# lh3/bwa

Measured on NVIDIA H100. Metric: reads_per_sec, higher is better.
Workload: dtype int32

## Files before the change

### bwa_b200/csrc/cuda/bwag_api.cu

```cuda
#include <stdio.h>
#include <stdlib.h>
#include <string.h>
#include <stdarg.h>
#include <pthread.h>
#include <time.h>
#include <math.h>
#include <sched.h>
#include "bwag_dev.cuh"
#include "bwag_kernels.h"

struct BlobHeader {
	u64 magic, primary, seq_len, bwt_size, n_sa, l_pac;
	u64 L2[5];
	u64 sa_shift;
	u64 off_bwt, off_sa, off_pac, total;
	u64 sb[BWAG_MAX_SB][4];
};
#define BLOB_MAGIC 0x3142574142323030ull
#define ALIGN256(x) (((x) + 255) & ~(size_t)255)

static __thread char g_err[512];
extern "C" const char *bwag_last_error(void) { return g_err[0] ? g_err : "no error"; }
static int set_err(const char *fmt, ...)
{
	va_list ap;
	va_start(ap, fmt);
	vsnprintf(g_err, sizeof(g_err), fmt, ap);
	va_end(ap);
	return 1;
}
int bwag_set_error(const char *msg) { return set_err("%s", msg); }
#define CK(call) do { cudaError_t e_ = (call); if (e_ != cudaSuccess) return set_err("%s failed at %s:%d: %s", #call, __FILE__, __LINE__, cudaGetErrorString(e_)); } while (0)
#define CKP(call) do { cudaError_t e_ = (call); if (e_ != cudaSuccess) { set_err("%s failed at %s:%d: %s", #call, __FILE__, __LINE__, cudaGetErrorString(e_)); return 0; } } while (0)

struct Counters {
	int next_read, next_task, max_rlen, next_read3;
	u64 next_seed;
	u64 n_intv, n_seeds;
	u64 occ_touches, sa_touches, ext_cells, glb_cells;
	u64 n_cig, n_md;
	u32 flags, n_pre;
	u64 t_dregs, t_tasks, t_max_z, t_text, t_complex;
	int t_max_lq, t_max_rl;
	int n_many;
	u32 n_swtasks;
};

struct DevBuf { void *p; size_t cap; };
static int buf_reserve(DevBuf *b, size_t bytes)
{
	if (bytes <= b->cap) return 0;
	if (b->p) cudaFree(b->p);
	b->p = 0; b->cap = 0;
	size_t want = bytes + bytes / 4 + 256;
	CK(cudaMalloc(&b->p, want));
	b->cap = want;
	return 0;
}
struct HostBuf { void *p; size_t cap; };
static int hbuf_reserve(HostBuf *b, size_t bytes)
{
	if (bytes <= b->cap) return 0;
	if (b->p) cudaFreeHost(b->p);
	b->p = 0; b->cap = 0;
	size_t want = bytes + bytes / 4 + 256;
	CK(cudaMallocHost(&b->p, want));
	b->cap = want;
	return 0;
}

struct bwag_ctx {
	int device, own_blob, n_sm;
	int imported;
	size_t map_bytes[3];
	void *blob;
	DevIndex ix;
	u64 *dense_sa;
	ulonglong2 *ktab;
	int baseline;
	cudaStream_t stream;
	cudaEvent_t ev0, ev1, ev_wait;
	Counters *d_cnt, *h_cnt;
	bwag_stats_t st;
	int sa_intv_disk;
	DevBuf s_k1, s_k1f, s_n3, s_eh, s_rseq, s_qseq, s_z, s_wcig, s_wmd, s_pack, s_zl;
	int grid_k1, grid_k1f, grid_k2, grid_k4, grid_k5;
#define N_SPARE 12
	struct bwag_batch *spare[N_SPARE];
	pthread_mutex_t mu;
	struct bwag_ctx *parent;
	void *d_tail; TailCtg tctg; const double *d_logtab; int have_ctg;
};

struct bwag_batch {
	bwag_ctx_t *ctx;
	bwag_ctx_t lc;
	int lc_ready;
	int n;
	i64 total_bases;
	int max_len;
	const i64 *h_off;
	DevBuf d_codes, d_off;
	DevBuf d_intv_beg, d_intv_n, d_intv, d_seed_beg, d_rbeg;
	HostBuf h_intv_beg, h_intv_n, h_intv, h_seed_beg, h_rbeg;
	DevBuf d_chain_off, d_chains, d_seeds, d_regs, d_nregs;
	DevBuf d_chain_beg, d_chain_cnt, d_reg_base, d_chain_rid, d_chain_frac, d_cregs, d_creg_beg, d_ctg;
	DevBuf s_bt, s_sn, s_ch, s_order, s_idx, s_keys;
	HostBuf h_regs, h_nregs, h_cregs, h_creg_beg, h_tmp;
	i64 n_intv, n_seeds;
	int seeded;
	DevBuf d_tasks, d_res, d_cig, d_md;
	HostBuf h_res, h_cig, h_md;
	DevBuf d_dregs, d_dreg_beg, d_dreg_n, d_task_beg, d_cflag, d_pe_is, d_rec, d_text, d_ptab;
	DevBuf d_swtasks, d_swres, d_swpool, d_swscratch; HostBuf h_swres;
	DevBuf d_hsp, d_flt_nchn; HostBuf h_hsp;
	DevBuf d_pre_n, d_pre_score, d_pre_cig;
	DevBuf d_sel;
	HostBuf h_pe_is, h_cflag, h_rec, h_text, h_ptab;
	int tail_ready;
	int regs_on_device;
};

static void batch_free(bwag_batch_t *b);
static void free_dev(DevBuf *b) { if (b->p) cudaFree(b->p); b->p = 0; b->cap = 0; }
static void free_host(HostBuf *b) { if (b->p) cudaFreeHost(b->p); b->p = 0; b->cap = 0; }

#ifndef BWAG_L2_FETCH_DEFAULT
#define BWAG_L2_FETCH_DEFAULT 0
#endif
#define K1_SMEM_MAX (200 * 1024)
#ifndef K1_COMPACT_DEFAULT
#define K1_COMPACT_DEFAULT 1
#endif
#ifdef BWAG_CUSIM
#define BWAG_KTAB_MAX_AUTO 5
#else
#define BWAG_KTAB_MAX_AUTO 14
#endif
#define K4_SMEM_MAX (96 * 1024)
#define K4L_SMEM_MAX (200 * 1024)
#define SEEDSW_MAXLEN 200

#ifdef BWAG_CUSIM
unsigned long long bwag_cusim_sector_loads, bwag_cusim_list_acc[5];
#endif


extern "C" size_t bwag_blob_bytes(const bwt_t *bwt, int64_t l_pac)
{
	return ALIGN256(sizeof(BlobHeader)) + ALIGN256((size_t)bwt->bwt_size * 4 + 64) + ALIGN256((size_t)bwt->n_sa * 8 + 32) + ALIGN256((size_t)l_pac / 4 + 1 + 64);
}

extern "C" int bwag_blob_fill(int device, void *d_blob, const bwt_t *bwt, int64_t l_pac, const uint8_t *pac)
{
	BlobHeader h;
	if (device >= 0) CK(cudaSetDevice(device));
	memset(&h, 0, sizeof(h));
	h.magic = BLOB_MAGIC; h.primary = bwt->primary; h.seq_len = bwt->seq_len; h.bwt_size = bwt->bwt_size; h.n_sa = bwt->n_sa; h.l_pac = (u64)l_pac;
	for (int i = 0; i < 5; ++i) h.L2[i] = bwt->L2[i];
	{
		int s = 0;
		while ((1 << s) < bwt->sa_intv) ++s;
		if ((1 << s) != bwt->sa_intv) return set_err("suffix-array interval %d is not a power of two", bwt->sa_intv);
		h.sa_shift = (u64)s;
	}
	if (bwt->seq_len >= (u64)BWAG_MAX_SB << BWAG_SB_SHIFT) return set_err("index too large: %llu BWT symbols", (unsigned long long)bwt->seq_len);
	for (u64 s = 0; s << BWAG_SB_SHIFT < bwt->seq_len; ++s) {
		const u64 *cnt = (const u64 *)(bwt->bwt + ((s << BWAG_SB_SHIFT) >> 7) * 16);
		for (int k = 0; k < 4; ++k) h.sb[s][k] = cnt[k];
// ... 400 lines not shown
	CKP(cudaMemcpyAsync(b->d_off.p, off, sizeof(i64) * ((size_t)n + 1), cudaMemcpyHostToDevice, c->stream));
	c->st.h2d_bytes += (u64)b->total_bases + sizeof(i64) * ((u64)n + 1);
	CKP(cudaEventRecord(c->ev1, c->stream));
	CKP(cudaStreamSynchronize(c->stream));
	{ float ms = 0; cudaEventElapsedTime(&ms, c->ev0, c->ev1); c->st.ms_h2d += ms; }
	return b;
}

extern "C" void bwag_batch_end(bwag_batch_t *b)
{
	if (!b) return;
	bwag_ctx_t *c = b->ctx;
	cudaSetDevice(c->device);
	cudaStreamSynchronize(b->lc.stream);
	pthread_mutex_lock(&c->mu);
	{
		bwag_stats_t *d = &c->st, *x = &b->lc.st;
		d->occ_touches += x->occ_touches; d->sa_touches += x->sa_touches; d->sa_touches_algo += x->sa_touches_algo;
		d->ext_cells += x->ext_cells; d->glb_cells += x->glb_cells;
		d->ms_smem += x->ms_smem; d->ms_sa += x->ms_sa; d->ms_chain += x->ms_chain; d->ms_extend += x->ms_extend; d->ms_global += x->ms_global;
		d->ms_h2d += x->ms_h2d; d->ms_d2h += x->ms_d2h; d->n_launch += x->n_launch; d->h2d_bytes += x->h2d_bytes; d->d2h_bytes += x->d2h_bytes;
		d->ms_tail += x->ms_tail; d->tail_reads += x->tail_reads; d->tail_complex += x->tail_complex; d->ms_localsw += x->ms_localsw; d->sw_tasks += x->sw_tasks;
	}
#ifdef BWAG_CUSIM
	if (getenv("BWA_B200_PROFILE")) fprintf(stderr, "[prof] emulator: %llu 32-byte block/table loads so far (K1, K1f, K2, table build); K1 candidate-list accesses by entry index 0-3: %llu, 4-7: %llu, 8-11: %llu, 12-15: %llu, 16+: %llu (the first K1_SLOTS of a list live in shared memory)\n", bwag_cusim_sector_loads, bwag_cusim_list_acc[0], bwag_cusim_list_acc[1], bwag_cusim_list_acc[2], bwag_cusim_list_acc[3], bwag_cusim_list_acc[4]);
#endif
	if (getenv("BWA_B200_PROFILE"))
		fprintf(stderr, "[prof] batch counters: %d reads, occ_touches %llu, sa_touches %llu, ext_cells %llu, glb_cells %llu; stage 4: %llu reads, %llu handed back to the host-side post-processing; K6: %llu local alignments\n", b->n,
		        (unsigned long long)b->lc.st.occ_touches, (unsigned long long)b->lc.st.sa_touches, (unsigned long long)b->lc.st.ext_cells, (unsigned long long)b->lc.st.glb_cells,
		        (unsigned long long)b->lc.st.tail_reads, (unsigned long long)b->lc.st.tail_complex, (unsigned long long)b->lc.st.sw_tasks);
	for (int i = 0; i < N_SPARE; ++i) if (!c->spare[i]) { c->spare[i] = b; b = 0; break; }
	pthread_mutex_unlock(&c->mu);
	if (b) batch_free(b);
}

static void batch_free(bwag_batch_t *b)
{
	if (b->lc_ready) {
		free_dev(&b->lc.s_pack); free_dev(&b->lc.s_k1); free_dev(&b->lc.s_k1f); free_dev(&b->lc.s_n3); free_dev(&b->lc.s_eh); free_dev(&b->lc.s_rseq); free_dev(&b->lc.s_qseq); free_dev(&b->lc.s_z); free_dev(&b->lc.s_wcig); free_dev(&b->lc.s_wmd);
		cudaFree(b->lc.d_cnt); cudaFreeHost(b->lc.h_cnt);
		cudaEventDestroy(b->lc.ev0); cudaEventDestroy(b->lc.ev1); cudaEventDestroy(b->lc.ev_wait); cudaStreamDestroy(b->lc.stream);
	}
	free_dev(&b->d_codes); free_dev(&b->d_off);
	free_dev(&b->d_intv_beg); free_dev(&b->d_intv_n); free_dev(&b->d_intv); free_dev(&b->d_seed_beg); free_dev(&b->d_rbeg);
	free_host(&b->h_intv_beg); free_host(&b->h_intv_n); free_host(&b->h_intv); free_host(&b->h_seed_beg); free_host(&b->h_rbeg);
	free_dev(&b->d_chain_off); free_dev(&b->d_chains); free_dev(&b->d_seeds); free_dev(&b->d_regs); free_dev(&b->d_nregs);
	free_dev(&b->d_chain_beg); free_dev(&b->d_chain_cnt); free_dev(&b->d_reg_base); free_dev(&b->d_chain_rid); free_dev(&b->d_chain_frac); free_dev(&b->d_cregs); free_dev(&b->d_creg_beg); free_dev(&b->d_ctg);
	free_dev(&b->s_bt); free_dev(&b->s_sn); free_dev(&b->s_ch); free_dev(&b->s_order); free_dev(&b->s_idx); free_dev(&b->s_keys);
	free_host(&b->h_regs); free_host(&b->h_nregs); free_host(&b->h_cregs); free_host(&b->h_creg_beg); free_host(&b->h_tmp);
	free_dev(&b->d_tasks); free_dev(&b->d_res); free_dev(&b->d_cig); free_dev(&b->d_md);
	free_host(&b->h_res); free_host(&b->h_cig); free_host(&b->h_md);
	free_dev(&b->d_sel); free_dev(&b->d_swtasks); free_dev(&b->d_swres); free_dev(&b->d_swpool); free_dev(&b->d_swscratch); free_host(&b->h_swres);
	free_dev(&b->d_hsp); free_dev(&b->d_flt_nchn); free_host(&b->h_hsp);
	free_dev(&b->d_pre_n); free_dev(&b->d_pre_score); free_dev(&b->d_pre_cig);
	free_dev(&b->d_dregs); free_dev(&b->d_dreg_beg); free_dev(&b->d_dreg_n); free_dev(&b->d_task_beg); free_dev(&b->d_cflag); free_dev(&b->d_pe_is); free_dev(&b->d_rec); free_dev(&b->d_text); free_dev(&b->d_ptab);
	free_host(&b->h_pe_is); free_host(&b->h_cflag); free_host(&b->h_rec); free_host(&b->h_text); free_host(&b->h_ptab);
	free(b);
}

static int reset_counters(bwag_ctx_t *c)
{
	CK(cudaMemsetAsync(c->d_cnt, 0, sizeof(Counters), c->stream));
	return 0;
}
static cudaError_t stream_wait(bwag_ctx_t *c)
{
	static int mode = -1;
	if (mode < 0) { const char *e = getenv("BWA_B200_SYNC"); mode = !e ? 3 : strcmp(e, "spin") == 0 ? 0 : strcmp(e, "block") == 0 ? 1 : strcmp(e, "yield") == 0 ? 2 : 3; }
	if (mode == 0) return cudaStreamSynchronize(c->stream);
	if (mode == 3) {
		long ns = 5000;
		for (;;) {
			cudaError_t q = cudaStreamQuery(c->stream);
			if (q != cudaErrorNotReady) return q;
			struct timespec ts = { 0, ns };
			nanosleep(&ts, 0);
			if (ns < 80000) ns <<= 1;
		}
	}
	if (mode == 2) {
		for (;;) {
			cudaError_t q = cudaStreamQuery(c->stream);
			if (q != cudaErrorNotReady) return q;
			sched_yield();
		}
	}
	cudaError_t e = cudaEventRecord(c->ev_wait, c->stream);
	if (e != cudaSuccess) return e;
	return cudaEventSynchronize(c->ev_wait);
}

static int fetch_counters(bwag_ctx_t *c)
{
	CK(cudaMemcpyAsync(c->h_cnt, c->d_cnt, sizeof(Counters), cudaMemcpyDeviceToHost, c->stream));
	CK(stream_wait(c));
	return 0;
}
#define H2D(c, dst, src, bytes) do { CK(cudaMemcpyAsync((dst), (src), (bytes), cudaMemcpyHostToDevice, (c)->stream)); (c)->st.h2d_bytes += (u64)(bytes); } while (0)
#define D2H(c, dst, src, bytes) do { CK(cudaMemcpyAsync((dst), (src), (bytes), cudaMemcpyDeviceToHost, (c)->stream)); (c)->st.d2h_bytes += (u64)(bytes); } while (0)
static double elapsed_at(bwag_ctx_t *c, const char *stage, int line)
{
	float ms = 0;
	cudaEventElapsedTime(&ms, c->ev0, c->ev1);
	if (g_gputrace > 0) {
		float t0 = 0, t1 = 0;
		cudaEventElapsedTime(&t0, g_trace_ref, c->ev0); cudaEventElapsedTime(&t1, g_trace_ref, c->ev1);
		fprintf(stderr, "[gputrace] %p %s:%d %.3f %.3f\n", (void *)c, stage, line, t0, t1);
// ... 505 lines not shown
	c->st.ms_d2h += elapsed_at(c, "d2h", __LINE__);
	out->n_regs = (const int32_t *)b->h_nregs.p; out->reg_beg = (const int64_t *)b->h_creg_beg.p; out->regs = (const bwag_creg_t *)b->h_cregs.p;
	return 0;
}


static int run_global(bwag_batch_t *b, const bwag_sw_par_t *par, int n_tasks, int cap_q, int cap_r, i64 cap_z, i64 n_aln, i64 *nc_out, i64 *nm_out)
{
	bwag_ctx_t *c = &b->lc;
	cap_q = (cap_q + 3) & ~3; cap_r = (cap_r + 15) & ~15; cap_z = (cap_z + 15) & ~(i64)15;
	if (cap_q < 4) cap_q = 4;
	if (cap_r < 16) cap_r = 16;
	if (cap_z < 64) cap_z = 64;
	const int cap_wcig = cap_q + cap_r + 4, cap_wmd = 3 * cap_r + cap_q + 16;
	int grid = c->grid_k5;
	const int k5_zsm = getenv("BWA_B200_K5_ZSM") ? atoi(getenv("BWA_B200_K5_ZSM")) & ~15 : 6144;
	const int k5_per_warp = ((8 * (cap_q + 2) + cap_r + cap_q + 2 + 15) & ~15) + k5_zsm;
	const size_t k5_smem = (size_t)k5_per_warp * (K5_THREADS / 32);
	int k5_sm = k5_smem <= K4_SMEM_MAX && !(getenv("BWA_B200_K5_SM") && atoi(getenv("BWA_B200_K5_SM")) == 0);
	const int k5_fast = !c->baseline && !(getenv("BWA_B200_K5_FAST") && atoi(getenv("BWA_B200_K5_FAST")) == 0);
#ifndef BWAG_CUSIM
	if (k5_sm) { int nb = 0; CK(cudaOccupancyMaxActiveBlocksPerMultiprocessor(&nb, k5_fast ? k_global_sm_fast : k_global_sm, K5_THREADS, k5_smem)); if (nb < 2) k5_sm = 0; else grid = c->n_sm * nb; }
#endif
	{
		i64 need = ((i64)n_tasks + (K5_THREADS / 32) - 1) / (K5_THREADS / 32);
		if (grid > need) grid = (int)(need > 0 ? need : 1);
		i64 max_warps = ((i64)8 << 30) / cap_z;
		if (max_warps < K5_THREADS / 32) max_warps = K5_THREADS / 32;
		if ((i64)grid * (K5_THREADS / 32) > max_warps) grid = (int)(max_warps / (K5_THREADS / 32));
	}
	const size_t n_warps = (size_t)grid * (K5_THREADS / 32);
	if (buf_reserve(&c->s_eh, n_warps * 2 * (size_t)(cap_q + 2) * 4) || buf_reserve(&c->s_rseq, n_warps * (size_t)cap_r) ||
	    buf_reserve(&c->s_qseq, n_warps * (size_t)(cap_q + 2)) || buf_reserve(&c->s_z, n_warps * (size_t)cap_z) ||
	    buf_reserve(&c->s_wcig, n_warps * (size_t)cap_wcig * 4) || buf_reserve(&c->s_wmd, n_warps * (size_t)cap_wmd)) return 1;
	if (buf_reserve(&b->d_res, sizeof(bwag_gres_t) * (size_t)n_tasks)) return 1;
	int k5_lane = !c->baseline && cap_q <= K5L_QWORDS * 4 && n_tasks >= 64 && getenv("BWA_B200_K5_LANE") && atoi(getenv("BWA_B200_K5_LANE")) != 0;
	const size_t k5l_smem = (size_t)K5L_RING * K5L_THREADS * 8 + (size_t)K5L_QWORDS * K5L_THREADS * 4;
	const i64 k5l_cap_z = (i64)(K5L_RING - 1) * (cap_r < 1024 ? cap_r : 1024);
	int k5l_grid = 0;
	if (k5_lane) {
#ifndef BWAG_CUSIM
		int nb = 0;
		CK(cudaFuncSetAttribute(k_global_lane, cudaFuncAttributeMaxDynamicSharedMemorySize, (int)k5l_smem));
		CK(cudaOccupancyMaxActiveBlocksPerMultiprocessor(&nb, k_global_lane, K5L_THREADS, k5l_smem));
		k5l_grid = c->n_sm * (nb > 0 ? nb : 1);
#else
		k5l_grid = 2;
#endif
		const i64 need = ((i64)n_tasks + K5L_THREADS - 1) / K5L_THREADS;
		if (k5l_grid > need) k5l_grid = (int)need;
		if (buf_reserve(&b->d_pre_n, 4 * (size_t)n_tasks) || buf_reserve(&b->d_pre_score, 4 * (size_t)n_tasks) || buf_reserve(&b->d_pre_cig, 4 * (size_t)K5L_MAXCIG * (size_t)n_tasks) ||
		    buf_reserve(&c->s_zl, (size_t)k5l_cap_z * (size_t)k5l_grid * K5L_THREADS)) return 1;
	}
	i64 cap_cig = n_aln * 6 + 1024, cap_md = n_aln * 24 + 4096;
	for (int attempt = 0;; ++attempt) {
		if (buf_reserve(&b->d_cig, 4 * (size_t)cap_cig) || buf_reserve(&b->d_md, (size_t)cap_md)) return 1;
		GlbArgs a;
		memset(&a, 0, sizeof(a));
		a.codes = (const uint8_t *)b->d_codes.p; a.off = (const i64 *)b->d_off.p; a.par = *par;
		a.tasks = (const bwag_gtask_t *)b->d_tasks.p; a.n_tasks = n_tasks;
		a.res = (bwag_gres_t *)b->d_res.p; a.cigar = (u32 *)b->d_cig.p; a.md = (char *)b->d_md.p;
		a.cap_cig = cap_cig; a.cap_md = cap_md; a.n_cig = &c->d_cnt->n_cig; a.n_md = &c->d_cnt->n_md;
		a.w_cig = (u32 *)c->s_wcig.p; a.w_md = (char *)c->s_wmd.p; a.cap_wcig = cap_wcig; a.cap_wmd = cap_wmd;
		a.eh = (int *)c->s_eh.p; a.rseq = (uint8_t *)c->s_rseq.p; a.qseq = (uint8_t *)c->s_qseq.p; a.z = (uint8_t *)c->s_z.p;
		a.cap_q = cap_q; a.cap_r = cap_r; a.cap_z = cap_z;
		a.next_task = &c->d_cnt->next_task; a.cells = &c->d_cnt->glb_cells; a.flags = &c->d_cnt->flags;
		if (reset_counters(c)) return 1;
		CK(cudaEventRecord(c->ev0, c->stream));
		if (k5_lane) {
			GlbLaneArgs la;
			memset(&la, 0, sizeof(la));
			la.codes = a.codes; la.off = a.off; la.par = *par; la.tasks = a.tasks; la.n_tasks = n_tasks;
			la.pre_n = (int *)b->d_pre_n.p; la.pre_score = (int *)b->d_pre_score.p; la.pre_cig = (u32 *)b->d_pre_cig.p;
			la.z = (uint8_t *)c->s_zl.p; la.cap_z = k5l_cap_z; la.next_task = &c->d_cnt->next_task; la.cells = &c->d_cnt->glb_cells; la.n_pre = &c->d_cnt->n_pre;
			BWAG_LAUNCH(k_global_lane, k5l_grid, K5L_THREADS, k5l_smem, c->stream, c->ix, la);
			CK(cudaGetLastError());
			CK(cudaMemsetAsync(&c->d_cnt->next_task, 0, sizeof(int), c->stream));
			a.pre_n = la.pre_n; a.pre_score = la.pre_score; a.pre_cig = la.pre_cig;
			++c->st.n_launch;
		}
		a.smem_per_warp = k5_sm ? k5_per_warp : 0; a.z_sm_bytes = k5_sm ? k5_zsm : 0;
		if (k5_sm && k5_fast) BWAG_LAUNCH(k_global_sm_fast, grid, K5_THREADS, k5_smem, c->stream, c->ix, a);
		else if (k5_sm) BWAG_LAUNCH(k_global_sm, grid, K5_THREADS, k5_smem, c->stream, c->ix, a);
		else if (k5_fast) BWAG_LAUNCH(k_global_fast, grid, K5_THREADS, 0, c->stream, c->ix, a);
		else BWAG_LAUNCH(k_global, grid, K5_THREADS, 0, c->stream, c->ix, a);
		CK(cudaGetLastError());
		CK(cudaEventRecord(c->ev1, c->stream));
		if (fetch_counters(c)) return 1;
		c->st.ms_global += elapsed_at(c, "global", __LINE__); ++c->st.n_launch;
		if (k5_lane && getenv("BWA_B200_PROFILE")) fprintf(stderr, "[prof] global alignment: lane-per-request kernel made %u of %d CIGARs, grid %d x %d\n", c->h_cnt->n_pre, n_tasks, k5l_grid, K5L_THREADS);
		if (c->h_cnt->flags & 4u) return set_err("global alignment: a task exceeded the scratch capacity");
		if (!(c->h_cnt->flags & 16u)) break;
		if (attempt >= 3) return set_err("global alignment: output pools keep overflowing");
		cap_cig = (i64)c->h_cnt->n_cig + 1024; cap_md = (i64)c->h_cnt->n_md + 4096;
	}
	c->st.glb_cells += c->h_cnt->glb_cells;
	*nc_out = (i64)c->h_cnt->n_cig; *nm_out = (i64)c->h_cnt->n_md;
	return 0;
}

extern "C" int bwag_global(bwag_batch_t *b, const bwag_sw_par_t *par, int n_tasks, const bwag_gtask_t *tasks, bwag_galn_t *out)
{
	bwag_ctx_t *c = &b->lc;
	CK(cudaSetDevice(c->device));
	if (n_tasks <= 0) { out->res = 0; out->cigar = 0; out->md = 0; return 0; }
	i64 cap_z = 64, n_aln = 0, nc = 0, nm = 0;
	int cap_q = 4, cap_r = 16;
	for (int t = 0; t < n_tasks; ++t) {
		i64 lq = tasks[t].qe - tasks[t].qb, rl = tasks[t].re - tasks[t].rb;
		if (lq > cap_q) cap_q = (int)lq;
		if (rl > cap_r) cap_r = (int)rl;
		if (tasks[t].mode == BWAG_G_REG2ALN) {
			i64 d = rl > lq ? rl - lq : lq - rl, wmax = (i64)par->w << 2;
			if (d + 3 > wmax) wmax = d + 3;
			i64 ncol = lq < 2 * wmax + 1 ? lq : 2 * wmax + 1;
			if (ncol * rl > cap_z) cap_z = ncol * rl;
			++n_aln;
		}
	}
	if (buf_reserve(&b->d_tasks, sizeof(bwag_gtask_t) * (size_t)n_tasks)) return 1;
	CK(cudaEventRecord(c->ev0, c->stream));
	H2D(c, b->d_tasks.p, tasks, sizeof(bwag_gtask_t) * (size_t)n_tasks);
	CK(cudaEventRecord(c->ev1, c->stream));
	CK(stream_wait(c));
	c->st.ms_h2d += elapsed_at(c, "h2d", __LINE__);
	b->tail_ready = 0;
	if (run_global(b, par, n_tasks, cap_q, cap_r, cap_z, n_aln, &nc, &nm)) return 1;
	if (hbuf_reserve(&b->h_res, sizeof(bwag_gres_t) * (size_t)n_tasks) || hbuf_reserve(&b->h_cig, 4 * (size_t)(nc + 1)) || hbuf_reserve(&b->h_md, (size_t)nm + 16)) return 1;
	CK(cudaEventRecord(c->ev0, c->stream));
	D2H(c, b->h_res.p, b->d_res.p, sizeof(bwag_gres_t) * (size_t)n_tasks);
	if (nc) D2H(c, b->h_cig.p, b->d_cig.p, 4 * (size_t)nc);
	if (nm) D2H(c, b->h_md.p, b->d_md.p, (size_t)nm);
	CK(cudaEventRecord(c->ev1, c->stream));
	CK(stream_wait(c));
	c->st.ms_d2h += elapsed_at(c, "d2h", __LINE__);
	out->res = (const bwag_gres_t *)b->h_res.p; out->cigar = (const uint32_t *)b->h_cig.p; out->md = (const char *)b->h_md.p;
	return 0;
}


#define TAIL_LOGN 4096
extern "C" int bwag_ctx_set_contigs(bwag_ctx_t *c, int n_seqs, const int64_t *offset, const int32_t *len, const uint8_t *is_alt, const char *const *names)
{
// ... 156 lines not shown
```

### bwa_b200/csrc/cuda/bwag_global.cu

```cuda
#include "bwag_dev.cuh"
#include "bwag_kernels.h"

#define NEG_INF (-0x40000000)

__device__ __forceinline__ int warp_ksw_global(int lane, int qlen, const uint8_t *q, int tlen, const uint8_t *t, const int8_t *mat,
                               int o_del, int e_del, int o_ins, int e_ins, int w, int *H, int *E, uint8_t *z, int n_col, u64 *cells)
{
	const int oe_del = o_del + e_del, oe_ins = o_ins + e_ins;
	for (int j = lane; j <= qlen; j += 32) {
		H[j] = j == 0 ? 0 : (j <= w ? -(o_ins + e_ins * j) : NEG_INF);
		E[j] = NEG_INF;
	}
	__syncwarp();
	for (int i = 0; i < tlen; ++i) {
		const int8_t *srow = mat + t[i] * 5;
		const int beg = i > w ? i - w : 0, end = i + w + 1 < qlen ? i + w + 1 : qlen;
		int carry_h = beg == 0 ? -(o_del + e_del * (i + 1)) : NEG_INF;
		int carry_f = NEG_INF;
		uint8_t *zi = z ? z + (i64)i * n_col : 0;
		if (end > beg) *cells += (u64)(end - beg);
		for (int j0 = beg; j0 < end; j0 += 32) {
			const int j = j0 + lane;
			const bool act = j < end;
			int m = NEG_INF, e = NEG_INF, tt, s, f, h, hp;
// ... 90 lines not shown
		}
		if (lane0) A::st_he(he + 8 * end, carry_h, NEG_INF);
		__syncwarp();
	}
	return A::ld_he(he + 8 * qlen).x;
}

__device__ __forceinline__ int md_put_num(char *md, int l, int v)
{
	char buf[12];
	int n = 0;
	do { buf[n++] = (char)('0' + v % 10); v /= 10; } while (v);
	while (n) md[l++] = buf[--n];
	return l;
}

template <bool C, class X, class Y> struct SelG { typedef X type; };
template <class X, class Y> struct SelG<false, X, Y> { typedef Y type; };

template <bool SM, bool FAST>
__device__ __forceinline__ void global_body(const DevIndex &ix, const GlbArgs &a)
{
	const int lane = threadIdx.x & 31;
	const i64 wid = ((i64)blockIdx.x * blockDim.x + threadIdx.x) >> 5;
	int *H, *E;
	uint8_t *rseq, *qseq, *z_glob = a.z + wid * a.cap_z, *z_sm = 0;
	if (SM) {
#ifdef BWAG_CUSIM
		unsigned char *dyn = cusim_dyn_smem;
#else
		extern __shared__ int4 k5_dyn[];
		unsigned char *dyn = reinterpret_cast<unsigned char *>(k5_dyn);
#endif
		unsigned char *mine = dyn + (size_t)(threadIdx.x >> 5) * a.smem_per_warp;
		H = reinterpret_cast<int *>(mine); E = H + a.cap_q + 2;
		rseq = reinterpret_cast<uint8_t *>(E + a.cap_q + 2);
		qseq = rseq + a.cap_r;
		if (a.z_sm_bytes) z_sm = mine + a.smem_per_warp - a.z_sm_bytes;
	} else {
		H = a.eh + wid * (i64)(2 * (a.cap_q + 2)); E = H + a.cap_q + 2;
		rseq = a.rseq + wid * (i64)a.cap_r; qseq = a.qseq + wid * (i64)(a.cap_q + 2);
	}
	typedef typename SelG<SM, SmemAcc, PtrAcc>::type A;
	typename A::addr he_a = A::make(H), rs_a = A::make(rseq), q_a = A::make(qseq);
	if constexpr (SM && FAST) { BWAG_KEEP(he_a); BWAG_KEEP(rs_a); BWAG_KEEP(q_a); }
	const bwag_sw_par_t &p = a.par;
	__shared__ int8_t s_mat[32];
	if (threadIdx.x < 25) s_mat[threadIdx.x] = p.mat[threadIdx.x];
	__syncthreads();
	typename SmemAcc::addr mat_a = SmemAcc::make(s_mat);
	if constexpr (FAST) BWAG_KEEP(mat_a);
	u64 cells = 0;
	int overflow = 0;

	for (;;) {
		int tix = 0;
		if (lane == 0) tix = atomicAdd(a.next_task, 1);
		tix = __shfl_sync(FULL_MASK, tix, 0);
		if (tix >= a.n_tasks) break;
		const bwag_gtask_t tk = a.tasks[tix];
		const int lq = tk.qe - tk.qb;
		const i64 rb = tk.rb, re = tk.re;
		u32 *cig = a.w_cig + wid * (i64)a.cap_wcig;
		char *md = a.w_md + wid * (i64)a.cap_wmd;
		int score = 0, n_cigar = 0, NM = -1, l_md = 0;
		bool ok = !(lq <= 0 || rb >= re || (rb < ix.l_pac && re > ix.l_pac)) && rb >= 0 && re <= ix.l_pac << 1;
		const int rlen = (int)(re - rb);
		if (ok && (lq > a.cap_q || rlen > a.cap_r)) { ok = false; overflow |= 4; }
		if (ok) {
			const uint8_t *query = a.codes + a.off[tk.read] + tk.qb;
			const bool rev = rb >= ix.l_pac;
			__syncwarp();
			for (int x = lane; x < rlen; x += 32) rseq[rev ? rlen - 1 - x : x] = (uint8_t)bwag_ref_base(ix, rb + x);
			for (int x = lane; x < lq; x += 32) qseq[rev ? lq - 1 - x : x] = query[x];
			__syncwarp();
			const int want = tk.mode == BWAG_G_REG2ALN;
			int w2 = tk.w, it = 0, last_sc = -(1 << 30);
			const bool have_pre = a.pre_n && a.pre_n[tix] >= 0;
			for (;;) {
				if (want) w2 = w2 < p.w << 2 ? w2 : p.w << 2;
				n_cigar = 0;
				if (have_pre) {
					score = a.pre_score[tix]; n_cigar = a.pre_n[tix];
					for (int x = lane; x < n_cigar; x += 32) cig[x] = a.pre_cig[(i64)tix * K5L_MAXCIG + x];
					__syncwarp();
				} else if (lq == rlen && w2 == 0) {
					int sc = 0;
					for (int x = lane; x < lq; x += 32) sc += s_mat[rseq[x] * 5 + qseq[x]];
					score = __reduce_add_sync(FULL_MASK, sc);
					if (want) { cig[0] = (u32)lq << 4; n_cigar = 1; }
				} else {
					int w, max_gap, max_ins, max_del, min_w, d = rlen - lq;
					d = d < 0 ? -d : d;
					max_ins = (int)((double)(((lq + 1) >> 1) * s_mat[0] - p.o_ins) / p.e_ins + 1.);
					max_del = (int)((double)(((lq + 1) >> 1) * s_mat[0] - p.o_del) / p.e_del + 1.);
					max_gap = max_ins > max_del ? max_ins : max_del;
					max_gap = max_gap > 1 ? max_gap : 1;
					w = (max_gap + d + 1) >> 1;
					w = w < w2 ? w : w2;
					min_w = d + 3;
					w = w > min_w ? w : min_w;
					const int n_col = lq < 2 * w + 1 ? lq : 2 * w + 1;
					if (want && (i64)n_col * rlen > a.cap_z) { overflow |= 4; score = 0; break; }
					uint8_t *z = z_sm && (i64)n_col * rlen <= a.z_sm_bytes ? z_sm : z_glob;
					if constexpr (FAST) score = warp_ksw_global_fast<A, SmemAcc>(lane, lq, q_a, rlen, rs_a, mat_a, p.o_del, p.e_del, p.o_ins, p.e_ins, w, he_a, want ? z : 0, n_col, &cells);
					else score = warp_ksw_global(lane, lq, qseq, rlen, rseq, s_mat, p.o_del, p.e_del, p.o_ins, p.e_ins, w, H, E, want ? z : 0, n_col, &cells);
					if (want) {
						if (lane == 0) {
							int i = rlen - 1, k = (i + w + 1 < lq ? i + w + 1 : lq) - 1, which = 0, n = 0, run_op = -1, run_len = 0;
#define K5_PUSH(op_, len_) do { if ((op_) == run_op) run_len += (len_); else { if (run_op >= 0) cig[n++] = (u32)run_len << 4 | (u32)run_op; run_op = (op_); run_len = (len_); } } while (0)
							while (i >= 0 && k >= 0) {
								which = z[(i64)i * n_col + (k - (i > w ? i - w : 0))] >> (which << 1) & 3;
// ... 95 lines not shown
```

### bwa_b200/csrc/cuda/bwag_global_lane.cu

```cuda
#include "bwag_dev.cuh"
#include "bwag_kernels.h"

#define NEG_INF (-0x40000000)

__global__ void __launch_bounds__(K5L_THREADS, 2) k_global_lane(DevIndex ix, GlbLaneArgs a)
{
#ifdef BWAG_CUSIM
	unsigned char *dyn = cusim_dyn_smem;
#else
	extern __shared__ int4 k5l_dyn[];
	unsigned char *dyn = reinterpret_cast<unsigned char *>(k5l_dyn);
#endif
	int2 *ring = reinterpret_cast<int2 *>(dyn) + threadIdx.x;
	u32 *qw = reinterpret_cast<u32 *>(dyn + (size_t)K5L_RING * K5L_THREADS * 8) + threadIdx.x;
	__shared__ int8_t s_mat[32];
	const bwag_sw_par_t &p = a.par;
	if (threadIdx.x < 25) s_mat[threadIdx.x] = p.mat[threadIdx.x];
	__syncthreads();
	const int lane = threadIdx.x & 31;
	const i64 wid = ((i64)blockIdx.x * blockDim.x + threadIdx.x) >> 5;
	uint8_t *z = a.z + wid * a.cap_z * 32 + lane;
	const int oe_del = p.o_del + p.e_del, oe_ins = p.o_ins + p.e_ins;
	u64 cells = 0;
	u32 n_pre = 0;
// ... 77 lines not shown
						t = m - oe_del;
						e -= p.e_del;
						d |= e > t ? 1 << 2 : 0;
						e = e > t ? e : t;
						*pe = make_int2(h1, e);
						h1 = h;
						t = m - oe_ins;
						f -= p.e_ins;
						d |= f > t ? 2 << 4 : 0;
						f = f > t ? f : t;
						zi[(i64)j * 32] = d;
					}
				}
				if (on) ring[(end & (K5L_RING - 1)) * K5L_THREADS] = make_int2(h1, NEG_INF);
			}
			if (live) score = ring[(lq & (K5L_RING - 1)) * K5L_THREADS].x;
			{
				int i = rlen - 1, k = (i + w + 1 < lq ? i + w + 1 : lq) - 1, which = 0, n = 0, run_op = -1, run_len = 0;
				bool fits = true;
#define K5L_PUSH(op_, len_) do { if ((op_) == run_op) run_len += (len_); else { if (run_op >= 0) { if (n < K5L_MAXCIG) cig[n] = (u32)run_len << 4 | (u32)run_op; else fits = false; ++n; } run_op = (op_); run_len = (len_); } } while (0)
				while (__any_sync(FULL_MASK, live && i >= 0 && k >= 0)) {
					if (live && i >= 0 && k >= 0) {
						which = z[((i64)i * n_col + (k - (i > w ? i - w : 0))) * 32] >> (which << 1) & 3;
						if (which == 0) { K5L_PUSH(0, 1); --i; --k; }
						else if (which == 1) { K5L_PUSH(2, 1); --i; }
						else { K5L_PUSH(1, 1); --k; }
					}
				}
				if (live) {
					if (i >= 0) K5L_PUSH(2, i + 1);
					if (k >= 0) K5L_PUSH(1, k + 1);
					if (run_op >= 0) { if (n < K5L_MAXCIG) cig[n] = (u32)run_len << 4 | (u32)run_op; else fits = false; ++n; }
					if (!fits) live = false;
					else {
						for (int x = 0; x < n >> 1; ++x) { const u32 tmp = cig[x]; cig[x] = cig[n - 1 - x]; cig[n - 1 - x] = tmp; }
						n_cig = n;
					}
				}
#undef K5L_PUSH
			}
			if (live) {
				bool more = !(score == last_sc || w2 == p.w << 2);
				if (more) { last_sc = score; w2 <<= 1; more = ++it < 3 && score < tk.truesc - p.a; }
				if (!more) {
					a.pre_n[tix] = n_cig; a.pre_score[tix] = score; ++n_pre;
					live = false;
				}
			}
		}
	}
	if (cells) atomicAdd(a.cells, cells);
	if (n_pre) atomicAdd(a.n_pre, n_pre);
}
```

### bwa_b200/csrc/cuda/bwag_kernels.h

```cpp
#ifndef BWAG_KERNELS_H
#define BWAG_KERNELS_H
#include "bwag_dev.cuh"

#define K1_THREADS 128
#define K1F_THREADS 128
#ifndef K1_SLOTS
#ifdef K1_PACKED8
#define K1_SLOTS 8
#else
#define K1_SLOTS 4
#endif
#endif
#define K1C_SLOTS 8
#define K1B_THREADS 128
#define K2_THREADS 128
#define K3_THREADS 128
#define K4_THREADS 128
#define K5_THREADS 128
#define K4L_THREADS 128
#ifndef K4L_MINB
#define K4L_MINB 3
#endif

struct Intv;
// ... 14 lines not shown
	const u32 *hasn;
	i64 *intv_beg; int *intv_n; bwtintv_t *intv; i64 *seed_beg; i64 *rbeg;
	i64 cap_intv, cap_seeds;
	int *next_read; u64 *n_intv; u64 *n_seeds; u64 *occ_touches; u32 *flags;
};

struct SaArgs { i64 *rbeg; i64 n; u64 *next; u64 *sa_touches; };

struct ChainArgs {
	const i64 *off; int n_reads;
	const i64 *intv_beg; const int *intv_n; const bwtintv_t *intv; const i64 *seed_beg; const i64 *rbeg;
	int w, max_chain_gap, max_occ, min_seed_len, min_chain_weight, max_chain_extend; float mask_level, drop_ratio;
	int a, o_del, e_del, o_ins, e_ins;
	i64 l_pac; int n_seqs; const i64 *ctg_off; const int *ctg_len; const uint8_t *ctg_alt;
	void *s_bt, *s_sn, *s_ch; int *s_order, *s_idx; u64 *s_keys;
	bwag_xchain_t *xchains; bwag_xseed_t *xseeds; int *chain_rid; float *chain_frac;
	i64 *chain_beg, *reg_base; int *n_chains;
	int *max_rlen;
	int *n_many; int many;
	const int *hsp_tab; bwag_swtask_t *sw_tasks; u32 *n_swtasks; const bwag_swres_t *sw_res; int *flt_nchn;
};

struct RegCompactArgs {
	int n_reads; const int *n_regs; const bwag_xreg_t *regs; const i64 *reg_base, *chain_beg; const int *chain_rid; const float *chain_frac;
	i64 *out_beg; bwag_creg_t *out; u64 *total;
};

struct ExtArgs {
	const uint8_t *codes; const i64 *off; int n_reads;
	bwag_sw_par_t par;
	const i64 *chain_beg; const int *chain_cnt; const i64 *reg_base;
	const bwag_xchain_t *chains; const bwag_xseed_t *seeds;
	bwag_xreg_t *regs; int32_t *n_regs;
	int *eh; uint8_t *rseq; int cap_q, cap_r;
	int smem_per_warp;
	int min_seed;
	int chain_lo, chain_hi;
	int *next_read; u64 *cells; u32 *flags;
};

struct GlbArgs {
	const uint8_t *codes; const i64 *off;
	bwag_sw_par_t par;
	const bwag_gtask_t *tasks; int n_tasks;
	bwag_gres_t *res; u32 *cigar; char *md;
	i64 cap_cig, cap_md; u64 *n_cig, *n_md;
	u32 *w_cig; char *w_md; int cap_wcig, cap_wmd;
	int *eh; uint8_t *rseq; uint8_t *qseq; uint8_t *z;
	int cap_q, cap_r; i64 cap_z;
	int smem_per_warp;
	int z_sm_bytes;
	int *next_task; u64 *cells; u32 *flags;
	const int *pre_n, *pre_score; const u32 *pre_cig;
};

#define K5L_THREADS 128
#define K5L_RING 64
#define K5L_QWORDS 64
#define K5L_MAXCIG 16
struct GlbLaneArgs {
	const uint8_t *codes; const i64 *off;
	bwag_sw_par_t par;
	const bwag_gtask_t *tasks; int n_tasks;
	int *pre_n, *pre_score; u32 *pre_cig;
	uint8_t *z; i64 cap_z;
	int *next_task; u64 *cells; u32 *n_pre;
};

struct TailCtg { i64 l_pac; int n_seqs; const i64 *off; const int *len; const uint8_t *alt; const char *names; const int *name_off; };

struct TailRegsArgs {
	int n_reads, pe;
	mem_opt_t opt;
	TailCtg ctg;
	const int *n_raw; const bwag_xreg_t *xregs; const i64 *reg_base, *chain_beg; const int *chain_rid; const float *chain_frac;
	mem_alnreg_t *dregs; i64 *dreg_beg; int *dreg_n; i64 *task_beg; uint8_t *cflag; i64 cap_dregs;
	bwag_gtask_t *tasks; i64 cap_tasks;
	u64 *pe_is;
	u64 *n_dregs, *n_tasks, *max_z; int *max_lq, *max_rl;
};

struct TailSamArgs {
	int n_reads, pe;
	mem_opt_t opt;
	TailCtg ctg;
	mem_pestat_t pes[4];
	const double *ptab[4];
	const double *logtab;
	i64 n_processed;
	const uint8_t *codes; const i64 *off;
	const mem_alnreg_t *dregs; const i64 *dreg_beg; const int *dreg_n; const i64 *task_beg; const uint8_t *cflag;
	const bwag_gres_t *res; const u32 *cigar; const char *md;
	const char *rg; int l_rg;
	bwag_samrec_t *rec; char *text; i64 cap_text; u64 *n_text, *n_complex;
};

struct SwArgs {
	const bwag_swtask_t *tasks; int n_tasks;
	bwag_sw_par_t par;
	const uint8_t *codes;
	const uint8_t *pool;
	bwag_swres_t *res;
	unsigned char *scratch; i64 per_thread; int cap_n, cap_q, cap_t;
	int *next_task; u32 *flags;
};

__global__ void k_chain_emit(ChainArgs a);
__global__ void k_global_lane(DevIndex ix, GlbLaneArgs a);
__global__ void k_localsw(DevIndex ix, SwArgs a);
__global__ void k_localsw_warp(DevIndex ix, SwArgs a);
__global__ void k_occ_pack(DevIndex ix, uint4 *bwt, u64 n_blocks);
__global__ void k_ktab_build(DevIndex ix, ulonglong2 *tab, int K);
__global__ void k_pack_reads(const uint8_t *codes, const i64 *off, int n_reads, u32 *packed, u32 *nmask, u32 *hasn);
__global__ void k_smem(DevIndex ix, SeedArgs a);
#ifndef K1_PACKED8
__global__ void k_smem_c(DevIndex ix, SeedArgs a);
#endif
__global__ void k_smem_fwd(DevIndex ix, SeedArgs a);
__global__ void k_seed_post(SeedArgs a);
__global__ void k_sa(DevIndex ix, SaArgs a);
__global__ void k_sa_densify(DevIndex ix, u64 *out, int out_shift, u64 n_out);
__global__ void k_index_verify(DevIndex ix, u64 first, u64 stride, u64 n_check, u64 *out);
__global__ void k_chain(ChainArgs a);
__global__ void k_regs_compact(RegCompactArgs a);
__global__ void k_regs_compact_sel(RegCompactArgs a, const int *sel, int n_sel, int *out_n);
__global__ void k_extend(DevIndex ix, ExtArgs a);
__global__ void k_extend_sm(DevIndex ix, ExtArgs a);
__global__ void k_extend_fast(DevIndex ix, ExtArgs a);
__global__ void k_extend_sm_fast(DevIndex ix, ExtArgs a);
__global__ void k_extend_lane(DevIndex ix, ExtArgs a);
__global__ void k_global(DevIndex ix, GlbArgs a);
__global__ void k_global_sm(DevIndex ix, GlbArgs a);
__global__ void k_global_fast(DevIndex ix, GlbArgs a);
__global__ void k_global_sm_fast(DevIndex ix, GlbArgs a);
__global__ void k_tail_regs(TailRegsArgs a);
__global__ void k_tail_sam(TailSamArgs g);

#endif
```

Baseline: 12.28 million.

## Split global alignment into gap-free lane kernel and warp kernel for the rest

```diff
diff --git a/bwa_b200/csrc/cuda/bwag_api.cu b/bwa_b200/csrc/cuda/bwag_api.cu
--- a/bwa_b200/csrc/cuda/bwag_api.cu
+++ b/bwa_b200/csrc/cuda/bwag_api.cu
@@ -40,6 +40,7 @@
 	u64 occ_touches, sa_touches, ext_cells, glb_cells;
 	u64 n_cig, n_md;
 	u32 flags, n_pre;
+	u32 k5_n[K5C_N];
 	u64 t_dregs, t_tasks, t_max_z, t_text, t_complex;
 	int t_max_lq, t_max_rl;
 	int n_many;
@@ -115,6 +116,7 @@
 	DevBuf d_swtasks, d_swres, d_swpool, d_swscratch; HostBuf h_swres;
 	DevBuf d_hsp, d_flt_nchn; HostBuf h_hsp;
 	DevBuf d_pre_n, d_pre_score, d_pre_cig;
+	DevBuf d_k5list;
 	DevBuf d_sel;
 	HostBuf h_pe_is, h_cflag, h_rec, h_text, h_ptab;
 	int tail_ready;
@@ -621,7 +623,7 @@
 	free_host(&b->h_res); free_host(&b->h_cig); free_host(&b->h_md);
 	free_dev(&b->d_sel); free_dev(&b->d_swtasks); free_dev(&b->d_swres); free_dev(&b->d_swpool); free_dev(&b->d_swscratch); free_host(&b->h_swres);
 	free_dev(&b->d_hsp); free_dev(&b->d_flt_nchn); free_host(&b->h_hsp);
-	free_dev(&b->d_pre_n); free_dev(&b->d_pre_score); free_dev(&b->d_pre_cig);
+	free_dev(&b->d_pre_n); free_dev(&b->d_pre_score); free_dev(&b->d_pre_cig); free_dev(&b->d_k5list);
 	free_dev(&b->d_dregs); free_dev(&b->d_dreg_beg); free_dev(&b->d_dreg_n); free_dev(&b->d_task_beg); free_dev(&b->d_cflag); free_dev(&b->d_pe_is); free_dev(&b->d_rec); free_dev(&b->d_text); free_dev(&b->d_ptab);
 	free_host(&b->h_pe_is); free_host(&b->h_cflag); free_host(&b->h_rec); free_host(&b->h_text); free_host(&b->h_ptab);
 	free(b);
@@ -1233,6 +1235,19 @@
 		if (buf_reserve(&b->d_pre_n, 4 * (size_t)n_tasks) || buf_reserve(&b->d_pre_score, 4 * (size_t)n_tasks) || buf_reserve(&b->d_pre_cig, 4 * (size_t)K5L_MAXCIG * (size_t)n_tasks) ||
 		    buf_reserve(&c->s_zl, (size_t)k5l_cap_z * (size_t)k5l_grid * K5L_THREADS)) return 1;
 	}
+	const int k5_split = !c->baseline && !k5_lane && k5_sm && k5_fast && cap_q <= K5L_QWORDS * 4 && !(getenv("BWA_B200_K5_SPLIT") && atoi(getenv("BWA_B200_K5_SPLIT")) == 0);
+	int gf_grid = 0;
+	if (k5_split) {
+		if (buf_reserve(&b->d_k5list, 4 * (size_t)K5C_N * (size_t)n_tasks)) return 1;
+#ifndef BWAG_CUSIM
+		int nb = 0;
+		CK(cudaOccupancyMaxActiveBlocksPerMultiprocessor(&nb, k_global_gapfree, 128, 0));
+		gf_grid = c->n_sm * (nb > 0 ? nb : 1);
+#else
+		gf_grid = 2;
+#endif
+		if (gf_grid > (n_tasks + 127) / 128) gf_grid = (n_tasks + 127) / 128;
+	}
 	i64 cap_cig = n_aln * 6 + 1024, cap_md = n_aln * 24 + 4096;
 	for (int attempt = 0;; ++attempt) {
 		if (buf_reserve(&b->d_cig, 4 * (size_t)cap_cig) || buf_reserve(&b->d_md, (size_t)cap_md)) return 1;
@@ -1260,6 +1275,19 @@
 			a.pre_n = la.pre_n; a.pre_score = la.pre_score; a.pre_cig = la.pre_cig;
 			++c->st.n_launch;
 		}
+		if (k5_split) {
+			int *lists = (int *)b->d_k5list.p;
+			GlbSplitArgs s;
+			memset(&s, 0, sizeof(s));
+			s.codes = a.codes; s.off = a.off; s.par = *par; s.tasks = a.tasks; s.n_tasks = n_tasks;
+			s.lists = lists; s.n = c->d_cnt->k5_n;
+			s.res = a.res; s.cigar = a.cigar; s.md = a.md; s.cap_cig = cap_cig; s.cap_md = cap_md; s.n_cig = a.n_cig; s.n_md = a.n_md; s.flags = a.flags;
+			BWAG_LAUNCH(k_global_classify, (n_tasks + 127) / 128, 128, 0, c->stream, c->ix, s);
+			BWAG_LAUNCH(k_global_gapfree, gf_grid, 128, 0, c->stream, c->ix, s);
+			CK(cudaGetLastError());
+			a.list = lists + (i64)K5C_WARP * n_tasks; a.list_n = c->d_cnt->k5_n + K5C_WARP;
+			c->st.n_launch += 2;
+		}
 		a.smem_per_warp = k5_sm ? k5_per_warp : 0; a.z_sm_bytes = k5_sm ? k5_zsm : 0;
 		if (k5_sm && k5_fast) BWAG_LAUNCH(k_global_sm_fast, grid, K5_THREADS, k5_smem, c->stream, c->ix, a);
 		else if (k5_sm) BWAG_LAUNCH(k_global_sm, grid, K5_THREADS, k5_smem, c->stream, c->ix, a);
@@ -1270,6 +1298,8 @@
 		if (fetch_counters(c)) return 1;
 		c->st.ms_global += elapsed_at(c, "global", __LINE__); ++c->st.n_launch;
 		if (k5_lane && getenv("BWA_B200_PROFILE")) fprintf(stderr, "[prof] global alignment: lane-per-request kernel made %u of %d CIGARs, grid %d x %d\n", c->h_cnt->n_pre, n_tasks, k5l_grid, K5L_THREADS);
+		if (k5_split && getenv("BWA_B200_PROFILE"))
+			fprintf(stderr, "[prof] global alignment: %d requests: %u gap-free by lane, %u by warp\n", n_tasks, c->h_cnt->k5_n[K5C_GAPFREE], c->h_cnt->k5_n[K5C_WARP]);
 		if (c->h_cnt->flags & 4u) return set_err("global alignment: a task exceeded the scratch capacity");
 		if (!(c->h_cnt->flags & 16u)) break;
 		if (attempt >= 3) return set_err("global alignment: output pools keep overflowing");
diff --git a/bwa_b200/csrc/cuda/bwag_global.cu b/bwa_b200/csrc/cuda/bwag_global.cu
--- a/bwa_b200/csrc/cuda/bwag_global.cu
+++ b/bwa_b200/csrc/cuda/bwag_global.cu
@@ -166,12 +166,14 @@
 	if constexpr (FAST) BWAG_KEEP(mat_a);
 	u64 cells = 0;
 	int overflow = 0;
+	const int n_all = a.list ? (int)*a.list_n : a.n_tasks;
 
 	for (;;) {
 		int tix = 0;
 		if (lane == 0) tix = atomicAdd(a.next_task, 1);
 		tix = __shfl_sync(FULL_MASK, tix, 0);
-		if (tix >= a.n_tasks) break;
+		if (tix >= n_all) break;
+		if (a.list) tix = a.list[tix];
 		const bwag_gtask_t tk = a.tasks[tix];
 		const int lq = tk.qe - tk.qb;
 		const i64 rb = tk.rb, re = tk.re;
diff --git a/bwa_b200/csrc/cuda/bwag_global_lane.cu b/bwa_b200/csrc/cuda/bwag_global_lane.cu
--- a/bwa_b200/csrc/cuda/bwag_global_lane.cu
+++ b/bwa_b200/csrc/cuda/bwag_global_lane.cu
@@ -153,3 +153,171 @@
 	if (cells) atomicAdd(a.cells, cells);
 	if (n_pre) atomicAdd(a.n_pre, n_pre);
 }
+
+
+__device__ __forceinline__ bool k5_window_ok(const DevIndex &ix, const bwag_gtask_t &tk)
+{
+	const int lq = tk.qe - tk.qb;
+	return !(lq <= 0 || tk.rb >= tk.re || (tk.rb < ix.l_pac && tk.re > ix.l_pac)) && tk.rb >= 0 && tk.re <= ix.l_pac << 1;
+}
+
+__device__ __forceinline__ i64 k5_fwd_start(const DevIndex &ix, const bwag_gtask_t &tk) { return tk.rb >= ix.l_pac ? (ix.l_pac << 1) - tk.re : tk.rb; }
+
+__device__ __forceinline__ int k5_md_num(char *md, int l, int v)
+{
+	char buf[12];
+	int n = 0;
+	do { buf[n++] = (char)('0' + v % 10); v /= 10; } while (v);
+	if (!md) return l + n;
+	while (n) md[l++] = buf[--n];
+	return l;
+}
+
+__device__ __forceinline__ void k5_reserve(int lane, int n_cig, int l_md, u64 *n_cig_ctr, u64 *n_md_ctr, i64 *co, i64 *mo)
+{
+	u32 c = (u32)n_cig, m = (u32)((l_md + 3) & ~3);
+#pragma unroll
+	for (int d = 1; d < 32; d <<= 1) {
+		const u32 vc = __shfl_up_sync(FULL_MASK, c, d), vm = __shfl_up_sync(FULL_MASK, m, d);
+		if (lane >= d) { c += vc; m += vm; }
+	}
+	u64 bc = 0, bm = 0;
+	if (lane == 31) { if (c) bc = atomicAdd(n_cig_ctr, (u64)c); if (m) bm = atomicAdd(n_md_ctr, (u64)m); }
+	bc = __shfl_sync(FULL_MASK, bc, 31); bm = __shfl_sync(FULL_MASK, bm, 31);
+	*co = (i64)(bc + c - (u32)n_cig); *mo = (i64)(bm + m - (u32)((l_md + 3) & ~3));
+}
+
+__global__ void __launch_bounds__(128) k_global_classify(DevIndex ix, GlbSplitArgs a)
+{
+	const int t = blockIdx.x * blockDim.x + threadIdx.x, lane = threadIdx.x & 31;
+	const bwag_sw_par_t &p = a.par;
+	int cls = t < a.n_tasks ? K5C_WARP : -1;
+	if (t < a.n_tasks) {
+		const bwag_gtask_t tk = a.tasks[t];
+		const int lq = tk.qe - tk.qb;
+		if (tk.mode == BWAG_G_REG2ALN && k5_window_ok(ix, tk) && lq == tk.re - tk.rb && (tk.w < p.w << 2 ? tk.w : p.w << 2) == 0
+		    && p.mat[0] == p.mat[6] && p.mat[0] == p.mat[12] && p.mat[0] == p.mat[18]) cls = K5C_GAPFREE;
+	}
+	for (int c = 0; c < K5C_N; ++c) {
+		const u32 m = __ballot_sync(FULL_MASK, cls == c);
+		if (!m) continue;
+		u32 base = 0;
+		if (lane == __ffs(m) - 1) base = atomicAdd(a.n + c, (u32)__popc(m));
+		base = __shfl_sync(FULL_MASK, base, __ffs(m) - 1);
+		if (cls == c) a.lists[(i64)c * a.n_tasks + base + __popc(m & ((1u << lane) - 1))] = t;
+	}
+}
+
+__device__ __forceinline__ u32 k5_pac_le(const uint8_t *pac, i64 wi)
+{
+	u32 v = reinterpret_cast<const u32 *>(pac)[wi];
+	v = (v >> 4 & 0x0f0f0f0fu) | (v & 0x0f0f0f0fu) << 4;
+	return (v >> 2 & 0x33333333u) | (v & 0x33333333u) << 2;
+}
+__device__ __forceinline__ u32 k5_ref16(const uint8_t *pac, i64 k)
+{
+	const i64 wi = k >> 4;
+	return __funnelshift_r(k5_pac_le(pac, wi), k5_pac_le(pac, wi + 1), (u32)(k & 15) << 1);
+}
+
+__device__ __forceinline__ void k5_ld16(const uint8_t *p, const uint8_t *lo, const uint8_t *hi, u32 o[4])
+{
+	const u32 *wp = reinterpret_cast<const u32 *>((uintptr_t)p & ~(uintptr_t)3);
+	const u32 sh = (u32)((uintptr_t)p & 3) << 3;
+	u32 v[5];
+#pragma unroll
+	for (int i = 0; i < 5; ++i) {
+		const uint8_t *wa = reinterpret_cast<const uint8_t *>(wp + i);
+		v[i] = wa + 4 > lo && wa < hi ? wp[i] : 0;
+	}
+#pragma unroll
+	for (int i = 0; i < 4; ++i) o[i] = __funnelshift_r(v[i], v[i + 1], sh);
+}
+
+__device__ __forceinline__ u32 k5_bswap(u32 v) { return v >> 24 | (v >> 8 & 0xff00u) | (v << 8 & 0xff0000u) | v << 24; }
+
+__device__ __forceinline__ u32 k5_mismatch16(const uint8_t *query, int lq, bool rev, u32 ref, int x0)
+{
+	u32 q[4];
+	if (!rev) k5_ld16(query + x0, query, query + lq, q);
+	else {
+		u32 r[4];
+		k5_ld16(query + lq - 16 - x0, query, query + lq, r);
+#pragma unroll
+		for (int i = 0; i < 4; ++i) q[i] = k5_bswap(r[3 - i]);
+	}
+	u32 mm = 0;
+#pragma unroll
+	for (int i = 0; i < 4; ++i) {
+		u32 r = ref >> (8 * i) & 0xffu;
+		r = (r | r << 12) & 0x000f000fu;
+		r = (r | r << 6) & 0x03030303u;
+		const u32 d = q[i] ^ r;
+		const u32 ne = (d | d >> 1 | d >> 2) & 0x01010101u;
+		mm |= ((ne * 0x00204081u) >> 21 & 0xfu) << (4 * i);
+	}
+	return mm;
+}
+
+__device__ __forceinline__ int k5_gapfree_walk(const DevIndex &ix, const uint8_t *query, int lq, bool rev, i64 F, const int8_t *mat, char *md, int *score, int *n_mm)
+{
+	int u = 0, l = 0, sc = 0, nm = 0;
+	for (int x0 = 0; x0 < lq; x0 += 16) {
+		const u32 ref = k5_ref16(ix.pac, F + x0) ^ (rev ? 0xffffffffu : 0u);
+		const int nv = lq - x0 < 16 ? lq - x0 : 16;
+		u32 mm = k5_mismatch16(query, lq, rev, ref, x0) & (nv == 16 ? 0xffffu : (1u << nv) - 1);
+		int done = 0;
+		sc += (nv - __popc(mm)) * mat[0];
+		while (mm) {
+			const int k = __ffs(mm) - 1;
+			const int rb = ref >> (2 * k) & 3, qb = query[rev ? lq - 1 - x0 - k : x0 + k];
+			sc += mat[rb * 5 + qb];
+			++nm;
+			l = k5_md_num(md, l, u + k - done);
+			if (md) md[l] = "ACGT"[rev ? 3 - rb : rb];
+			++l;
+			u = 0; done = k + 1;
+			mm &= mm - 1;
+		}
+		u += nv - done;
+	}
+	l = k5_md_num(md, l, u);
+	if (md) md[l] = 0;
+	*score = sc; *n_mm = nm;
+	return l + 1;
+}
+
+__global__ void __launch_bounds__(128) k_global_gapfree(DevIndex ix, GlbSplitArgs a)
+{
+	__shared__ int8_t s_mat[32];
+	if (threadIdx.x < 25) s_mat[threadIdx.x] = a.par.mat[threadIdx.x];
+	__syncthreads();
+	const int lane = threadIdx.x & 31;
+	const int n = (int)a.n[K5C_GAPFREE];
+	const int *list = a.lists + (i64)K5C_GAPFREE * a.n_tasks;
+	u32 overflow = 0;
+	for (int base = (blockIdx.x * blockDim.x + threadIdx.x) & ~31; base < n; base += gridDim.x * blockDim.x) {
+		const int idx = base + lane;
+		const bool live = idx < n;
+		const int t = live ? list[idx] : 0;
+		const bwag_gtask_t tk = a.tasks[t];
+		const int lq = live ? tk.qe - tk.qb : 0;
+		const bool rev = tk.rb >= ix.l_pac;
+		const i64 F = k5_fwd_start(ix, tk);
+		const uint8_t *query = a.codes + a.off[tk.read] + tk.qb;
+		int score = 0, nm = 0, l_md = 0;
+		if (live) l_md = k5_gapfree_walk(ix, query, lq, rev, F, s_mat, 0, &score, &nm);
+		i64 co, mo;
+		k5_reserve(lane, live ? 1 : 0, l_md, a.n_cig, a.n_md, &co, &mo);
+		if (live) {
+			if (co + 1 <= a.cap_cig && mo + l_md <= a.cap_md) {
+				a.cigar[co] = (u32)lq << 4;
+				k5_gapfree_walk(ix, query, lq, rev, F, s_mat, a.md + mo, &score, &nm);
+			} else overflow = 16;
+			bwag_gres_t r;
+			r.score = score; r.n_cigar = 1; r.NM = nm; r.l_md = l_md; r.cigar_off = co; r.md_off = mo;
+			a.res[t] = r;
+		}
+	}
+	if (overflow) atomicOr(a.flags, overflow);
+}
diff --git a/bwa_b200/csrc/cuda/bwag_kernels.h b/bwa_b200/csrc/cuda/bwag_kernels.h
--- a/bwa_b200/csrc/cuda/bwag_kernels.h
+++ b/bwa_b200/csrc/cuda/bwag_kernels.h
@@ -90,6 +90,7 @@
 	int z_sm_bytes;
 	int *next_task; u64 *cells; u32 *flags;
 	const int *pre_n, *pre_score; const u32 *pre_cig;
+	const int *list; const u32 *list_n;
 };
 
 #define K5L_THREADS 128
@@ -103,6 +104,15 @@
 	int *pre_n, *pre_score; u32 *pre_cig;
 	uint8_t *z; i64 cap_z;
 	int *next_task; u64 *cells; u32 *n_pre;
+};
+
+enum { K5C_GAPFREE = 0, K5C_WARP, K5C_N };
+struct GlbSplitArgs {
+	const uint8_t *codes; const i64 *off;
+	bwag_sw_par_t par;
+	const bwag_gtask_t *tasks; int n_tasks;
+	int *lists; u32 *n;
+	bwag_gres_t *res; u32 *cigar; char *md; i64 cap_cig, cap_md; u64 *n_cig, *n_md; u32 *flags;
 };
 
 struct TailCtg { i64 l_pac; int n_seqs; const i64 *off; const int *len; const uint8_t *alt; const char *names; const int *name_off; };
@@ -145,6 +155,8 @@
 
 __global__ void k_chain_emit(ChainArgs a);
 __global__ void k_global_lane(DevIndex ix, GlbLaneArgs a);
+__global__ void k_global_classify(DevIndex ix, GlbSplitArgs a);
+__global__ void k_global_gapfree(DevIndex ix, GlbSplitArgs a);
 __global__ void k_localsw(DevIndex ix, SwArgs a);
 __global__ void k_localsw_warp(DevIndex ix, SwArgs a);
 __global__ void k_occ_pack(DevIndex ix, uint4 *bwt, u64 n_blocks);
```

Measured after the change: 12.44 million, median of 6. +1.2%, better.
